# shuhan-wang1/SNLP---Tenary-Post-train-Quantization

Hardware: AMD Instinct MI355X
Metric: weight-columns quantized/sec (and s/layer) at d=4096 (higher is better)
Workload: dtype fp16->f32

## Files before the change

snlp---tenary-post-train-quantization_amd/csrc/ef.hip:

```cpp
#include "common.hpp"
#include "internal.hpp"
#include "probe.hpp"

namespace {

typedef float f32x16 __attribute__((ext_vector_type(16)));
typedef float f32x4 __attribute__((ext_vector_type(4)));
typedef unsigned u32x4 __attribute__((ext_vector_type(4)));

constexpr int EF_T = 128;
constexpr int EF_ROWB = EF_T * 4;
constexpr int E2_KS = 32;
constexpr int E2_PANEL = E2_KS * EF_ROWB;
constexpr int E2_STAGE = 2 * E2_PANEL;
constexpr int EF_CV = 16;
constexpr unsigned EF_DROP = 0x80000000u;

__device__ uint4 ef_zero16;

PT2Q_DEV int ef_wave() { return (int)(threadIdx.x >> 6); }

struct EfArgs {
  const float* Ck;
  long ldk;
  const float* Et;
  float* Wt;
  long ldw;
  const int* crow;
  int nr, bs, te, ti, ntile;
  long zs;
  int nz;
  float* part;
  int n;
};

PT2Q_DEV EfArgs ef_linear(const EfArgs& a0, int z) {
  EfArgs a = a0;
  const long o = (long)z * a0.zs;
  a.Ck = (const float*)((const char*)a0.Ck + o);
  a.Et = (const float*)((const char*)a0.Et + o);
  a.Wt = (float*)((char*)a0.Wt + o);
  a.crow = (const int*)((const char*)a0.crow + o);
  if (a0.part) a.part = (float*)((char*)a0.part + o);
  return a;
}

PT2Q_DEV void ef_dma_asm(const char* sbase, uint32_t voff, uint32_t m0) {
  asm volatile("s_mov_b32 m0, %2\n\ts_nop 0\n\tglobal_load_lds_dwordx4 %0, %1" ::"v"(voff), "s"(sbase), "s"(m0)
               : "memory");
}

template <int OFF>
PT2Q_DEV float ef_ld(uint32_t addr) {
  float r;
  asm volatile("ds_read_b32 %0, %1 offset:%2" : "=v"(r) : "v"(addr), "i"(OFF));
  return r;
}

template <int N>
PT2Q_DEV void ef_wait(float (&a)[2], float (&b)[2]) {
  asm volatile("s_waitcnt lgkmcnt(%4)" : "+v"(a[0]), "+v"(a[1]), "+v"(b[0]), "+v"(b[1]) : "n"(N));
}

template <int S>
PT2Q_DEV void ef_read(uint32_t baseA, uint32_t baseB, float (&a)[2], float (&b)[2]) {
  a[0] = ef_ld<S * 2 * EF_ROWB>(baseA);
  a[1] = ef_ld<S * 2 * EF_ROWB + 128>(baseA);
  b[0] = ef_ld<S * 2 * EF_ROWB>(baseB);
  b[1] = ef_ld<S * 2 * EF_ROWB + 128>(baseB);
}

struct EfAcc {
  f32x16 acc[2][2];

  template <int S>
  PT2Q_DEV void run(uint32_t bA, uint32_t bB, float (&a)[4][2], float (&b)[4][2]) {
    constexpr int NP = E2_KS / 2;
    if constexpr (S < NP) {
      constexpr int c = S % 4;
      if constexpr (S + 2 < NP) ef_read<S + 2>(bA, bB, a[(S + 2) % 4], b[(S + 2) % 4]);
      if constexpr (S > 0) {
        constexpr int p = (S + 3) % 4;
        asm volatile("" ::"v"(a[p][0]), "v"(a[p][1]), "v"(b[p][0]), "v"(b[p][1]));
      }
      __builtin_amdgcn_sched_barrier(0);
      acc[0][0] = __builtin_amdgcn_mfma_f32_32x32x2f32(b[c][0], a[c][0], acc[0][0], 0, 0, 0);
      __builtin_amdgcn_sched_barrier(0);
      acc[0][1] = __builtin_amdgcn_mfma_f32_32x32x2f32(b[c][1], a[c][0], acc[0][1], 0, 0, 0);
      __builtin_amdgcn_sched_barrier(0);
      acc[1][0] = __builtin_amdgcn_mfma_f32_32x32x2f32(b[c][0], a[c][1], acc[1][0], 0, 0, 0);
      __builtin_amdgcn_sched_barrier(0);
      acc[1][1] = __builtin_amdgcn_mfma_f32_32x32x2f32(b[c][1], a[c][1], acc[1][1], 0, 0, 0);
      __builtin_amdgcn_sched_barrier(0);
      if constexpr (S + 1 < NP) {
        ef_wait<(S + 2 < NP ? 4 : 0)>(a[(S + 1) % 4], b[(S + 1) % 4]);
      }
      run<S + 1>(bA, bB, a, b);
    }
  }

  PT2Q_DEV void stage(uint32_t stg) {
    const int lane = threadIdx.x & 63, wave = ef_wave();
    const int wr = wave >> 1, wc = wave & 1, li = lane & 31, lk = lane >> 5;
    const uint32_t bA = stg + lk * EF_ROWB + (wr * 64 + li) * 4;
    const uint32_t bB = stg + E2_PANEL + lk * EF_ROWB + (wc * 64 + li) * 4;
    float a[4][2], b[4][2];
    ef_read<0>(bA, bB, a[0], b[0]);
    ef_read<1>(bA, bB, a[1], b[1]);
    ef_wait<4>(a[0], b[0]);
    run<0>(bA, bB, a, b);
  }
};

PT2Q_DEV int ef_row(int e0, int rm) {
  const int lane = threadIdx.x & 63, wr = ef_wave() >> 1;
  return e0 + wr * 64 + rm * 32 + (lane & 31);
}

PT2Q_DEV void ef_rowbase(const EfArgs& a, const int (&wrow)[2], int i0, uint32_t (&rb)[2]) {
  const int lane = threadIdx.x & 63, wc = ef_wave() & 1;
  const int i = i0 + wc * 64 + 4 * (lane >> 5);
#pragma unroll
  for (int rm = 0; rm < 2; ++rm)
    rb[rm] = (wrow[rm] < 0 || i0 + wc * 64 >= a.ldw || probe::ef_drop_wt)
                 ? EF_DROP
                 : (uint32_t)(((long)wrow[rm] * a.ldw + i) * 4);
}

PT2Q_DEV void ef_rows(const EfArgs& a, int e0, int (&wrow)[2]) {
  int v[2];
#pragma unroll
  for (int rm = 0; rm < 2; ++rm) {
    const int e = ef_row(e0, rm);
    v[rm] = a.crow[e < a.nr ? e : 0];
  }
#pragma unroll
  for (int rm = 0; rm < 2; ++rm) wrow[rm] = ef_row(e0, rm) < a.nr ? v[rm] : -1;
}

constexpr int EF_PS = 8;
constexpr int EF_RED = 512;

template <int J>
PT2Q_DEV void ef_wbar_step(const int (&prow)[2], const u32x4 (&pend)[EF_CV], float* red) {
  constexpr int rn = J >> 4, q = (J >> 2) & 3, u = J & 3;
  const int lane = threadIdx.x & 63, wave = ef_wave();
  const float v0 = prow[0] >= 0 ? __uint_as_float(pend[rn * 4 + q][u]) : 0.0f;
  const float v1 = prow[1] >= 0 ? __uint_as_float(pend[(2 + rn) * 4 + q][u]) : 0.0f;
  float x = bfly16(v0 + v1);
  x = x + __int_as_float(__builtin_amdgcn_update_dpp(0, __float_as_int(x), 0x142, 0xA, 0xF, false));
  const bool sel = (lane & 31) == 16;
  red[sel ? wave * 64 + (lane >> 5) * 32 + J : 256 + wave * 64 + lane] = x;
}

PT2Q_DEV void ef_wbar_store(int n, __amdgpu_buffer_rsrc_t rp, bool valid, int e0, int i0, const float* red) {
  const int lane = threadIdx.x & 63, wave = ef_wave(), wr = wave >> 1, wc = wave & 1;
  const int h = lane >> 5;
  const bool mine = valid && wr == 0 && (lane & 31) == 0;
  const long cb = (long)(e0 / EF_T) * n;
  const f32x4* X = (const f32x4*)(red + wc * 64 + h * 32);
  const f32x4* Y = (const f32x4*)(red + (wc + 2) * 64 + h * 32);
#pragma unroll
  for (int rn = 0; rn < 2; ++rn) {
    f32x4 x[4], y[4];
#pragma unroll
    for (int q = 0; q < 4; ++q) {
      x[q] = X[rn * 4 + q];
      y[q] = Y[rn * 4 + q];
    }
#pragma unroll
    for (int q = 0; q < 4; ++q) {
      const int i = i0 + wc * 64 + rn * 32 + 8 * q + 4 * h;
      const f32x4 o = x[q] + y[q];
      const unsigned off = (mine && i < n) ? (unsigned)((cb + i) * 4) : EF_DROP;
      __builtin_amdgcn_raw_buffer_store_b128(__builtin_bit_cast(u32x4, o), rp, off, 0, 0);
    }
  }
}


struct E2Vo {
  uint32_t a[4], b[4];
};

PT2Q_DEV void e2_voff(const EfArgs& a, E2Vo& v) {
  const int lane = threadIdx.x & 63, wave = ef_wave();
#pragma unroll
  for (int q = 0; q < 4; ++q) {
    const int kr = (wave * 4 + q) * 2 + (lane >> 5), d = 4 * (lane & 31);
    v.a[q] = (uint32_t)(((long)kr * a.ldk + d) * 4);
    v.b[q] = (uint32_t)(((long)kr * a.ldw + d) * 4);
  }
}

PT2Q_DEV void e2_stage_q(const EfArgs& a, int e0, int i0, int s, const char* ba, const char* bb, const E2Vo& v,
                         uint8_t* stg, int q, bool withB) {
  const int lane = threadIdx.x & 63, wave = ef_wave();
  typedef __attribute__((address_space(3))) void* lptr;
  const int k = s * E2_KS + (wave * 4 + q) * 2 + (lane >> 5);
  const int d = 4 * (lane & 31);
  const bool kin = k < a.bs;
  const void* sa = kin ? (const void*)(e0 + d < a.nr ? ba + v.a[q] : (const char*)a.Ck) : (const void*)&ef_zero16;
  const void* sb = kin ? (const void*)(i0 + d < a.ldw ? bb + v.b[q] : (const char*)a.Et) : (const void*)&ef_zero16;
  const int wv = __builtin_amdgcn_readfirstlane(wave);
  __builtin_amdgcn_global_load_lds(sa, (lptr)(stg + (wv * 4 + q) * 1024), 16, 0, 0);
  if (withB) __builtin_amdgcn_global_load_lds(sb, (lptr)(stg + E2_PANEL + (wv * 4 + q) * 1024), 16, 0, 0);
}

PT2Q_DEV int e2_stage(const EfArgs& a, int e0, int i0, int s, uint8_t* stg, uint32_t stg_lds, const E2Vo& v,
                      bool withB) {
  if constexpr ((PT2Q_EF2_KPROBE & 2) != 0) {
    typedef __attribute__((address_space(3))) void* lptr;
    const int wv = __builtin_amdgcn_readfirstlane(ef_wave());
#pragma unroll
    for (int q = 0; q < 4; ++q) {
      __builtin_amdgcn_global_load_lds(&ef_zero16, (lptr)(stg + (wv * 4 + q) * 1024), 16, 0, 0);
      if (withB) __builtin_amdgcn_global_load_lds(&ef_zero16, (lptr)(stg + E2_PANEL + (wv * 4 + q) * 1024), 16, 0, 0);
    }
    return withB ? 8 : 4;
  }
  const bool fast = (s + 1) * E2_KS <= a.bs && e0 + EF_T <= a.nr && i0 + EF_T <= a.ldw;
  const char* ba = (const char*)(a.Ck + (long)s * E2_KS * a.ldk + e0);
  const char* bb = (const char*)(a.Et + (long)s * E2_KS * a.ldw + i0);
  if (!fast) {
#pragma unroll
    for (int q = 0; q < 4; ++q) e2_stage_q(a, e0, i0, s, ba, bb, v, stg, q, withB);
    return withB ? 8 : 4;
  }
  const int wv = __builtin_amdgcn_readfirstlane(ef_wave());
  const uint32_t mA = stg_lds + (uint32_t)(wv * 4 * 1024), mB = mA + E2_PANEL;
#pragma unroll
  for (int q = 0; q < 4; ++q) {
    ef_dma_asm(ba, v.a[q], mA + q * 1024);
    if (withB) ef_dma_asm(bb, v.b[q], mB + q * 1024);
  }
  return withB ? 8 : 4;
}

PT2Q_DEV void e2_vmcnt(int n) {
  switch (n) {
#define E2_W(k) \
  case k: asm volatile("s_waitcnt vmcnt(" #k ")" ::: "memory"); break;
    E2_W(0) E2_W(1) E2_W(2) E2_W(3) E2_W(4) E2_W(5) E2_W(6) E2_W(7) E2_W(8) E2_W(9) E2_W(10) E2_W(11) E2_W(12)
    E2_W(13) E2_W(14) E2_W(15) E2_W(16) E2_W(17) E2_W(18) E2_W(19) E2_W(20) E2_W(21) E2_W(22) E2_W(23) E2_W(24)
    E2_W(25) E2_W(26) E2_W(27) E2_W(28) E2_W(29) E2_W(30) E2_W(31) E2_W(32) E2_W(33) E2_W(34) E2_W(35) E2_W(36)
    E2_W(37) E2_W(38) E2_W(39) E2_W(40) E2_W(41) E2_W(42) E2_W(43) E2_W(44) E2_W(45) E2_W(46) E2_W(47) E2_W(48)
    E2_W(49) E2_W(50) E2_W(51) E2_W(52) E2_W(53) E2_W(54) E2_W(55) E2_W(56) E2_W(57) E2_W(58) E2_W(59) E2_W(60)
    E2_W(61) E2_W(62)
#undef E2_W
    default: asm volatile("s_waitcnt vmcnt(0)" ::: "memory"); break;
  }
}

template <int J, int JE>
PT2Q_DEV void ef_wbar_span(const int (&prow)[2], const u32x4 (&pend)[EF_CV], float* red) {
  if constexpr (J < JE) {
    ef_wbar_step<J>(prow, pend, red);
    ef_wbar_span<J + 1, JE>(prow, pend, red);
  }
}

template <int RN>
PT2Q_DEV void e2_load(u32x4 (&c)[EF_CV], __amdgpu_buffer_rsrc_t rc, const uint32_t (&rb)[2]) {
#pragma unroll
  for (int rm = 0; rm < 2; ++rm)
#pragma unroll
    for (int q = 0; q < 4; ++q)
      c[(rm * 2 + RN) * 4 + q] = __builtin_amdgcn_raw_buffer_load_b128(rc, rb[rm] + 4 * (32 * RN + 8 * q), 0, 0);
}

template <int RN>
PT2Q_DEV void e2_sub(u32x4 (&c)[EF_CV], const EfAcc& F) {
#pragma unroll
  for (int rm = 0; rm < 2; ++rm)
#pragma unroll
    for (int q = 0; q < 4; ++q) {
      const int j = (rm * 2 + RN) * 4 + q;
#pragma unroll
      for (int u = 0; u < 4; ++u) c[j][u] = __float_as_uint(__uint_as_float(c[j][u]) - F.acc[rm][RN][4 * q + u]);
    }
}

template <int RN>
PT2Q_DEV void e2_store(const u32x4 (&c)[EF_CV], __amdgpu_buffer_rsrc_t rc, const uint32_t (&rb)[2]) {
#pragma unroll
  for (int rm = 0; rm < 2; ++rm)
#pragma unroll
    for (int q = 0; q < 4; ++q)
      __builtin_amdgcn_raw_buffer_store_b128(c[(rm * 2 + RN) * 4 + q], rc, rb[rm] + 4 * (32 * RN + 8 * q), 0,
                                             PT2Q_EF2_STORE_AUX);
}

PT2Q_DEV uint32_t e2_g1_chunk(int wv, int j) {
  return (uint32_t)(j < 4 ? (wv * 4 + j) * 1024 : E2_PANEL + (wv * 4 + j - 4) * 1024);
}
PT2Q_DEV void e2_g1_dma(__amdgpu_buffer_rsrc_t rc, const uint32_t (&rb)[2], uint8_t* slot) {
  typedef __attribute__((address_space(3))) void* lptr;
  const int lane = threadIdx.x & 63, wv = __builtin_amdgcn_readfirstlane(ef_wave());
#pragma unroll
  for (int j = 0; j < 8; ++j) {
    const uint32_t src = (uint32_t)__shfl((int)rb[j >> 2], 8 * (j & 3) + (lane >> 3));
    const uint32_t off = src == EF_DROP ? EF_DROP : src + 4 * (32 + 4 * (lane & 7));
    __builtin_amdgcn_raw_ptr_buffer_load_lds(rc, (lptr)(slot + e2_g1_chunk(wv, j)), 16, off, 0, 0, 0);
  }
}
PT2Q_DEV void e2_g1_read(u32x4 (&c)[EF_CV], const uint8_t* slot) {
  const int lane = threadIdx.x & 63, wv = __builtin_amdgcn_readfirstlane(ef_wave());
  const int li = lane & 31, h = lane >> 5;
#pragma unroll
  for (int rm = 0; rm < 2; ++rm)
#pragma unroll
    for (int q = 0; q < 4; ++q) {
      const int j = rm * 4 + (li >> 3), piece = ((li & 7) << 3) | (2 * q + h);
      c[(rm * 2 + 1) * 4 + q] = *(const u32x4*)(slot + e2_g1_chunk(wv, j) + 16 * piece);
    }
}

template <int NST>
__global__ __launch_bounds__(256) __attribute__((amdgpu_waves_per_eu(2, 2))) void ef2_gemm_kernel(
    EfArgs a0, long wt_bytes, long part_bytes) {
  static_assert(NST == 2 || NST == 4, "two or four K stages per tile");
  constexpr bool G1L = NST == 4;
  __shared__ __attribute__((aligned(1024))) uint8_t smem[2 * E2_STAGE];
  __shared__ __attribute__((aligned(16))) float red[EF_RED];
  const uint32_t lds0 = (uint32_t)(uintptr_t)(__attribute__((address_space(3))) uint8_t*)smem;
  const int total = a0.ntile * a0.nz;
  int t = (int)blockIdx.x;
  if (t >= total) return;
  PT2Q_EF2_CLK(0);
  auto corner = [&](int t, EfArgs& a, int& e0, int& i0) {
    const int z = t / a0.ntile, tl = t - z * a0.ntile;
    a = ef_linear(a0, z);
    e0 = (tl / a0.ti) * EF_T;
    i0 = (tl % a0.ti) * EF_T;
  };
  auto rsrc = [&](const EfArgs& a) { return __builtin_amdgcn_make_buffer_rsrc(a.Wt, 0, (int)wt_bytes, 0x00020000); };
  auto prsrc = [&](const EfArgs& x) { return __builtin_amdgcn_make_buffer_rsrc(x.part, 0, (int)part_bytes, 0x00020000); };
  const int P = a0.part ? EF_PS : 0;
  EfArgs a;
  int e0, i0, wrow[2];
  corner(t, a, e0, i0);
  asm volatile("s_waitcnt vmcnt(0) lgkmcnt(0)" ::: "memory");
  __syncthreads();
  ef_rows(a, e0, wrow);
  E2Vo vo;
  e2_voff(a0, vo);
  e2_stage(a, e0, i0, 0, smem, lds0, vo, true);
  int Dn1 = e2_stage(a, e0, i0, 1, smem + E2_STAGE, lds0 + E2_STAGE, vo, true);
  int SP = 0;
  int par = 0;
  constexpr int G0S = NST - 1 - PT2Q_EF2_G0_EARLY < 0 ? 0 : NST - 1 - PT2Q_EF2_G0_EARLY;
  for (;;) {
    const int tn = t + (int)gridDim.x;
    const bool more = tn < total;
    int en = e0, in = i0, nrow[2];
    EfArgs an = a;
    if (more) corner(tn, an, en, in);
    const bool newB = NST != 2 || !(more && an.Et == a.Et && in == i0);
    const __amdgpu_buffer_rsrc_t rc = rsrc(a);
    uint32_t rb[2];
    ef_rowbase(a, wrow, i0, rb);
    if constexpr ((PT2Q_EF2_KPROBE & 1) != 0) rb[0] = rb[1] = EF_DROP;
    uint32_t rbl[2] = {rb[0], rb[1]}, rbs[2] = {rb[0], rb[1]};
    if constexpr ((PT2Q_EF2_KPROBE & 8) != 0) rbl[0] = rbl[1] = 0;
    if constexpr ((PT2Q_EF2_KPROBE & 16) != 0) rbs[0] = rbs[1] = 0;
    ef_rows(an, en, nrow);
    EfAcc F;
#pragma unroll
    for (int rm = 0; rm < 2; ++rm)
#pragma unroll
      for (int rn = 0; rn < 2; ++rn) F.acc[rm][rn] = f32x16{};
    u32x4 c[EF_CV];
    int X[NST];
#pragma unroll
    for (int s = 0; s < NST; ++s) {
      const int young = s == 0   ? Dn1 + SP + 2
                        : s == 1 ? (G1L && SP > 0 ? SP - EF_CV / 2 : SP) + 2 + (G0S == 0 ? EF_CV / 2 : 0) + X[0]
                                 : X[s - 1];
      e2_vmcnt(young);
      asm volatile("s_barrier" ::: "memory");
      if (s == G0S) e2_load<0>(c, rc, rbl);
      const int sl = G1L ? (s + par) & 1 : s & 1;
      if constexpr ((PT2Q_EF2_KPROBE & 4) == 0) F.stage(lds0 + sl * E2_STAGE);
      asm volatile("s_waitcnt lgkmcnt(0)\n\ts_barrier" ::: "memory");
      uint8_t* slot = smem + sl * E2_STAGE;
      const uint32_t slot_lds = lds0 + sl * E2_STAGE;
      if (s + 2 < NST) {
        X[s] = e2_stage(a, e0, i0, s + 2, slot, slot_lds, vo, true);
      } else if (G1L && s == NST - 2) {
        e2_g1_dma(rc, rbl, slot);
        X[s] = EF_CV / 2;
      } else if (G1L) {
        X[s] = more ? e2_stage(an, en, in, 0, slot, slot_lds, vo, newB) : 0;
      } else if (more) {
        X[s] = e2_stage(an, en, in, s + 2 - NST, slot, slot_lds, vo, newB);
        if (s == NST - 1) Dn1 = X[s];
      } else {
        X[s] = 0;
      }
    }
    e2_vmcnt(X[NST - 1]);
    e2_sub<0>(c, F);
    if constexpr (!G1L) e2_load<1>(c, rc, rbl);
    e2_store<0>(c, rc, rbs);
    if (P) {
      asm volatile("s_waitcnt lgkmcnt(0)\n\ts_barrier" ::: "memory");
      ef_wbar_span<0, 16>(wrow, c, red);
    }
    if constexpr (G1L) {
      uint8_t* g1 = smem + par * E2_STAGE;
      e2_g1_read(c, g1);
      asm volatile("s_waitcnt lgkmcnt(0)" ::: "memory");
      Dn1 = more ? e2_stage(an, en, in, 1, g1, lds0 + par * E2_STAGE, vo, newB) : 0;
      par ^= 1;
    } else {
      e2_vmcnt(EF_CV / 2);
    }
    e2_sub<1>(c, F);
    e2_store<1>(c, rc, rbs);
    if (P) {
      ef_wbar_span<16, 32>(wrow, c, red);
      asm volatile("s_waitcnt lgkmcnt(0)\n\ts_barrier" ::: "memory");
      ef_wbar_store(a0.n, prsrc(a), true, e0, i0, red);
    }
    SP = EF_CV + P;
    if (!more) break;
    t = tn;
    a = an;
    e0 = en;
    i0 = in;
    wrow[0] = nrow[0];
    wrow[1] = nrow[1];
  }
  PT2Q_EF2_CLK(1);
}

}

int pt2q_launch_ef(const float* Ck, long ldk, const float* Et, float* Wt, long ldw, long wt_rows,
                   const int* crow, int nr, int bs, hipStream_t st, const Grp* grp, float* part, int n) {
  if (nr <= 0) return PT2Q_OK;
  const long wt_bytes = wt_rows * ldw * 4;
  const long part_bytes = part ? (long)ceil_div(nr, EF_T) * n * 4 : 0;
  if (bs <= 0 || bs > 4 * E2_KS || ldw % 4 || ldk % 4 || (uintptr_t)Ck % 16 || (uintptr_t)Et % 16 ||
      (uintptr_t)Wt % 16 || wt_bytes >= (long)EF_DROP || wt_rows > 65536)
    return PT2Q_E_UNSUPPORTED;
  if (part && (n <= 0 || n % 4 || n > ldw || (uintptr_t)part % 16 || part_bytes >= (long)EF_DROP))
    return PT2Q_E_UNSUPPORTED;
  EfArgs a{Ck, ldk, Et, Wt, ldw, crow, nr, bs, ceil_div(nr, EF_T), ceil_div(ldw, EF_T), 0,
           grp ? grp->ws : 0l, (int)grp_z(grp), part, n};
  a.ntile = a.te * a.ti;
  int dev = 0, cus = 256;
  if (hipGetDevice(&dev) == hipSuccess) (void)hipDeviceGetAttribute(&cus, hipDeviceAttributeMultiprocessorCount, dev);
  const int grid = std::min(a.ntile * a.nz, 2 * cus);
  if (bs <= 2 * E2_KS)
    hipLaunchKernelGGL(ef2_gemm_kernel<2>, dim3(grid), dim3(256), 0, st, a, wt_bytes, part_bytes);
  else
    hipLaunchKernelGGL(ef2_gemm_kernel<4>, dim3(grid), dim3(256), 0, st, a, wt_bytes, part_bytes);
  PT2Q_LAUNCH_CHECK();
  return PT2Q_OK;
}
```

Baseline: 516,000.

## Add register-resident E kernel with software-pipelined tile walk for large block sizes

```diff
diff --git a/snlp---tenary-post-train-quantization_amd/csrc/ef.hip b/snlp---tenary-post-train-quantization_amd/csrc/ef.hip
--- a/snlp---tenary-post-train-quantization_amd/csrc/ef.hip
+++ b/snlp---tenary-post-train-quantization_amd/csrc/ef.hip
@@ -139,7 +139,7 @@
 }
 
 constexpr int EF_PS = 8;
-constexpr int EF_RED = 512;
+constexpr int EF_RED = 544;
 
 template <int J>
 PT2Q_DEV void ef_wbar_step(const int (&prow)[2], const u32x4 (&pend)[EF_CV], float* red) {
@@ -150,7 +150,7 @@
   float x = bfly16(v0 + v1);
   x = x + __int_as_float(__builtin_amdgcn_update_dpp(0, __float_as_int(x), 0x142, 0xA, 0xF, false));
   const bool sel = (lane & 31) == 16;
-  red[sel ? wave * 64 + (lane >> 5) * 32 + J : 256 + wave * 64 + lane] = x;
+  (red + (sel ? wave * 64 + (lane >> 5) * 32 : 256 + wave * 64 + lane))[J] = x;
 }
 
 PT2Q_DEV void ef_wbar_store(int n, __amdgpu_buffer_rsrc_t rp, bool valid, int e0, int i0, const float* red) {
@@ -291,36 +291,9 @@
                                              PT2Q_EF2_STORE_AUX);
 }
 
-PT2Q_DEV uint32_t e2_g1_chunk(int wv, int j) {
-  return (uint32_t)(j < 4 ? (wv * 4 + j) * 1024 : E2_PANEL + (wv * 4 + j - 4) * 1024);
-}
-PT2Q_DEV void e2_g1_dma(__amdgpu_buffer_rsrc_t rc, const uint32_t (&rb)[2], uint8_t* slot) {
-  typedef __attribute__((address_space(3))) void* lptr;
-  const int lane = threadIdx.x & 63, wv = __builtin_amdgcn_readfirstlane(ef_wave());
-#pragma unroll
-  for (int j = 0; j < 8; ++j) {
-    const uint32_t src = (uint32_t)__shfl((int)rb[j >> 2], 8 * (j & 3) + (lane >> 3));
-    const uint32_t off = src == EF_DROP ? EF_DROP : src + 4 * (32 + 4 * (lane & 7));
-    __builtin_amdgcn_raw_ptr_buffer_load_lds(rc, (lptr)(slot + e2_g1_chunk(wv, j)), 16, off, 0, 0, 0);
-  }
-}
-PT2Q_DEV void e2_g1_read(u32x4 (&c)[EF_CV], const uint8_t* slot) {
-  const int lane = threadIdx.x & 63, wv = __builtin_amdgcn_readfirstlane(ef_wave());
-  const int li = lane & 31, h = lane >> 5;
-#pragma unroll
-  for (int rm = 0; rm < 2; ++rm)
-#pragma unroll
-    for (int q = 0; q < 4; ++q) {
-      const int j = rm * 4 + (li >> 3), piece = ((li & 7) << 3) | (2 * q + h);
-      c[(rm * 2 + 1) * 4 + q] = *(const u32x4*)(slot + e2_g1_chunk(wv, j) + 16 * piece);
-    }
-}
-
-template <int NST>
 __global__ __launch_bounds__(256) __attribute__((amdgpu_waves_per_eu(2, 2))) void ef2_gemm_kernel(
     EfArgs a0, long wt_bytes, long part_bytes) {
-  static_assert(NST == 2 || NST == 4, "two or four K stages per tile");
-  constexpr bool G1L = NST == 4;
+  constexpr int NST = 2;
   __shared__ __attribute__((aligned(1024))) uint8_t smem[2 * E2_STAGE];
   __shared__ __attribute__((aligned(16))) float red[EF_RED];
   const uint32_t lds0 = (uint32_t)(uintptr_t)(__attribute__((address_space(3))) uint8_t*)smem;
@@ -348,7 +321,6 @@
   e2_stage(a, e0, i0, 0, smem, lds0, vo, true);
   int Dn1 = e2_stage(a, e0, i0, 1, smem + E2_STAGE, lds0 + E2_STAGE, vo, true);
   int SP = 0;
-  int par = 0;
   constexpr int G0S = NST - 1 - PT2Q_EF2_G0_EARLY < 0 ? 0 : NST - 1 - PT2Q_EF2_G0_EARLY;
   for (;;) {
     const int tn = t + (int)gridDim.x;
@@ -356,7 +328,7 @@
     int en = e0, in = i0, nrow[2];
     EfArgs an = a;
     if (more) corner(tn, an, en, in);
-    const bool newB = NST != 2 || !(more && an.Et == a.Et && in == i0);
+    const bool newB = !(more && an.Et == a.Et && in == i0);
     const __amdgpu_buffer_rsrc_t rc = rsrc(a);
     uint32_t rb[2];
     ef_rowbase(a, wrow, i0, rb);
@@ -374,26 +346,17 @@
     int X[NST];
 #pragma unroll
     for (int s = 0; s < NST; ++s) {
-      const int young = s == 0   ? Dn1 + SP + 2
-                        : s == 1 ? (G1L && SP > 0 ? SP - EF_CV / 2 : SP) + 2 + (G0S == 0 ? EF_CV / 2 : 0) + X[0]
-                                 : X[s - 1];
+      const int young = s == 0 ? Dn1 + SP + 2 : SP + 2 + (G0S == 0 ? EF_CV / 2 : 0) + X[0];
       e2_vmcnt(young);
       asm volatile("s_barrier" ::: "memory");
       if (s == G0S) e2_load<0>(c, rc, rbl);
-      const int sl = G1L ? (s + par) & 1 : s & 1;
+      const int sl = s & 1;
       if constexpr ((PT2Q_EF2_KPROBE & 4) == 0) F.stage(lds0 + sl * E2_STAGE);
       asm volatile("s_waitcnt lgkmcnt(0)\n\ts_barrier" ::: "memory");
       uint8_t* slot = smem + sl * E2_STAGE;
       const uint32_t slot_lds = lds0 + sl * E2_STAGE;
-      if (s + 2 < NST) {
-        X[s] = e2_stage(a, e0, i0, s + 2, slot, slot_lds, vo, true);
-      } else if (G1L && s == NST - 2) {
-        e2_g1_dma(rc, rbl, slot);
-        X[s] = EF_CV / 2;
-      } else if (G1L) {
-        X[s] = more ? e2_stage(an, en, in, 0, slot, slot_lds, vo, newB) : 0;
-      } else if (more) {
-        X[s] = e2_stage(an, en, in, s + 2 - NST, slot, slot_lds, vo, newB);
+      if (more) {
+        X[s] = e2_stage(an, en, in, s, slot, slot_lds, vo, newB);
         if (s == NST - 1) Dn1 = X[s];
       } else {
         X[s] = 0;
@@ -401,21 +364,13 @@
     }
     e2_vmcnt(X[NST - 1]);
     e2_sub<0>(c, F);
-    if constexpr (!G1L) e2_load<1>(c, rc, rbl);
+    e2_load<1>(c, rc, rbl);
     e2_store<0>(c, rc, rbs);
     if (P) {
       asm volatile("s_waitcnt lgkmcnt(0)\n\ts_barrier" ::: "memory");
       ef_wbar_span<0, 16>(wrow, c, red);
     }
-    if constexpr (G1L) {
-      uint8_t* g1 = smem + par * E2_STAGE;
-      e2_g1_read(c, g1);
-      asm volatile("s_waitcnt lgkmcnt(0)" ::: "memory");
-      Dn1 = more ? e2_stage(an, en, in, 1, g1, lds0 + par * E2_STAGE, vo, newB) : 0;
-      par ^= 1;
-    } else {
-      e2_vmcnt(EF_CV / 2);
-    }
+    e2_vmcnt(EF_CV / 2);
     e2_sub<1>(c, F);
     e2_store<1>(c, rc, rbs);
     if (P) {
@@ -431,6 +386,320 @@
     i0 = in;
     wrow[0] = nrow[0];
     wrow[1] = nrow[1];
+  }
+  PT2Q_EF2_CLK(1);
+}
+
+constexpr int E3_NP = 64;
+constexpr int E3_APANEL = 4 * E2_PANEL;
+constexpr int E3_VM_TOP = EF_CV + EF_CV + EF_PS;
+constexpr int E3_VM_END = 2 + EF_CV + EF_CV + EF_CV + EF_PS;
+
+PT2Q_DEV void ef_dma_lane(const void* src, uint32_t m0) {
+  asm volatile("s_mov_b32 m0, %1\n\ts_nop 0\n\tglobal_load_lds_dwordx4 %0, off" ::"v"(src), "s"(m0) : "memory");
+}
+
+template <int J>
+PT2Q_DEV const void* e3_dma_src(const EfArgs& a, int e0, const E2Vo& v) {
+  constexpr int s = J >> 2, q = J & 3;
+  const int lane = threadIdx.x & 63, wave = ef_wave();
+  const int k = s * E2_KS + (wave * 4 + q) * 2 + (lane >> 5), d = 4 * (lane & 31);
+  const char* ba = (const char*)(a.Ck + (long)s * E2_KS * a.ldk + e0);
+  return k < a.bs ? (const void*)(e0 + d < a.nr ? ba + v.a[q] : (const char*)a.Ck) : (const void*)&ef_zero16;
+}
+template <int J>
+PT2Q_DEV void e3_dma(const void* src, uint32_t panel) {
+  constexpr int s = J >> 2, q = J & 3;
+  ef_dma_lane(src, panel + s * E2_PANEL + (uint32_t)((__builtin_amdgcn_readfirstlane(ef_wave()) * 4 + q) * 1024));
+}
+
+template <int J>
+PT2Q_DEV void e3_dma_all(const EfArgs& a, int e0, uint32_t panel, const E2Vo& v) {
+  if constexpr (J < 16) {
+    e3_dma<J>(e3_dma_src<J>(a, e0, v), panel);
+    e3_dma_all<J + 1>(a, e0, panel, v);
+  }
+}
+
+PT2Q_DEV float e3_ldg(u32x4 r, uint32_t off) {
+  float v;
+  asm volatile("buffer_load_dword %0, %1, %2, 0 offen" : "=a"(v) : "v"(off), "s"(r) : "memory");
+  return v;
+}
+
+PT2Q_DEV void e3_load_e(const EfArgs& a, int i0, float (&E)[2][E3_NP]) {
+  const int lane = threadIdx.x & 63, wc = ef_wave() & 1, li = lane & 31, lk = lane >> 5;
+  const uintptr_t p = (uintptr_t)a.Et;
+  u32x4 r;
+  r[0] = (unsigned)__builtin_amdgcn_readfirstlane((int)(uint32_t)p);
+  r[1] = (unsigned)__builtin_amdgcn_readfirstlane((int)(uint32_t)((p >> 32) & 0xffff));
+  r[2] = (unsigned)__builtin_amdgcn_readfirstlane((int)((long)a.bs * a.ldw * 4));
+  r[3] = 0x00020000u;
+  const uint32_t step = (uint32_t)(a.ldw * 8);
+#pragma unroll
+  for (int rn = 0; rn < 2; ++rn) {
+    const int col = i0 + wc * 64 + rn * 32 + li;
+    const uint32_t o0 = (uint32_t)(((long)lk * a.ldw + col) * 4);
+#pragma unroll
+    for (int pr = 0; pr < E3_NP; ++pr) {
+      E[rn][pr] = e3_ldg(r, (col < a.ldw && 2 * pr + lk < a.bs) ? o0 + pr * step : EF_DROP);
+      __builtin_amdgcn_sched_barrier(0);
+    }
+  }
+}
+
+PT2Q_DEV void e3_tie(float (&E)[2][E3_NP]) {
+#pragma unroll
+  for (int rn = 0; rn < 2; ++rn)
+#pragma unroll
+    for (int pr = 0; pr < E3_NP; ++pr) asm volatile("" : "+a"(E[rn][pr]));
+}
+
+PT2Q_DEV void e3_rows_issue(const EfArgs& a, int e0, int (&v)[2]) {
+#pragma unroll
+  for (int rm = 0; rm < 2; ++rm) {
+    const int e = ef_row(e0, rm);
+    asm volatile("global_load_dword %0, %1, off" : "=v"(v[rm]) : "v"(a.crow + (e < a.nr ? e : 0)) : "memory");
+  }
+}
+PT2Q_DEV void e3_rows_take(const EfArgs& a, int e0, int (&v)[2], int (&wrow)[2]) {
+  asm volatile("s_waitcnt vmcnt(%2)" : "+v"(v[0]), "+v"(v[1]) : "n"(2 * EF_CV));
+#pragma unroll
+  for (int rm = 0; rm < 2; ++rm) wrow[rm] = ef_row(e0, rm) < a.nr ? v[rm] : -1;
+}
+
+template <int IMM>
+PT2Q_DEV u32x4 e3_ld4(__amdgpu_buffer_rsrc_t r, uint32_t off) {
+  u32x4 v;
+  asm volatile("buffer_load_dwordx4 %0, %1, %2, 0 offen offset:%3" : "=v"(v) : "v"(off), "s"(r), "i"(IMM) : "memory");
+  return v;
+}
+PT2Q_DEV void e3_tie_old(u32x4 (&c)[EF_CV]) {
+#pragma unroll
+  for (int j = 0; j < EF_CV; ++j) asm volatile("" : "+v"(c[j]));
+}
+template <int J>
+PT2Q_DEV void e3_load_old(u32x4 (&c)[EF_CV], __amdgpu_buffer_rsrc_t rc, const uint32_t (&rb)[2]) {
+  if constexpr (J < EF_CV) {
+    constexpr int RN = J >> 3, rm = (J >> 2) & 1, q = J & 3;
+    c[(rm * 2 + RN) * 4 + q] = e3_ld4<4 * (32 * RN + 8 * q)>(rc, rb[rm]);
+    e3_load_old<J + 1>(c, rc, rb);
+  }
+}
+
+template <int N>
+PT2Q_DEV void e3_wait(float (&a)[2]) {
+  asm volatile("s_waitcnt lgkmcnt(%2)" : "+v"(a[0]), "+v"(a[1]) : "n"(N));
+}
+
+template <int P>
+PT2Q_DEV void e3_read(uint32_t bA, float (&a)[2]) {
+  a[0] = ef_ld<P * 2 * EF_ROWB>(bA);
+  a[1] = ef_ld<P * 2 * EF_ROWB + 128>(bA);
+}
+
+struct E3Tile {
+  int z, e0, i0;
+  int wrow[2];
+  uint32_t rb[2];
+};
+
+struct E3Jobs {
+  const EfArgs& a0;
+  const E2Vo& vo;
+  long wt_bytes, part_bytes;
+  float* red;
+  E3Tile prev, next;
+  bool more;
+  uint32_t panel;
+  int nrow[2];
+
+  PT2Q_DEV __amdgpu_buffer_rsrc_t wt(int z) const {
+    return __builtin_amdgcn_make_buffer_rsrc(ef_linear(a0, z < 0 ? 0 : z).Wt, 0, (int)wt_bytes, 0x00020000);
+  }
+
+  template <int P>
+  PT2Q_DEV void fold(u32x4 (&res)[EF_CV]) {
+    if constexpr (P < 32) ef_wbar_step<P>(prev.wrow, res, red);
+  }
+
+  template <int P>
+  PT2Q_DEV const void* prep() {
+    if constexpr (P < 16) return e3_dma_src<(P & 15)>(ef_linear(a0, next.z), next.e0, vo);
+    return nullptr;
+  }
+
+  template <int P>
+  PT2Q_DEV void mem(u32x4 (&res)[EF_CV], const void* src) {
+    constexpr int J = P & 15, RN = J >> 3, rm = (J >> 2) & 1, q = J & 3, idx = (rm * 2 + RN) * 4 + q;
+    constexpr int imm = 4 * (32 * RN + 8 * q);
+    if constexpr (P < 16) {
+      e3_dma<J>(src, panel);
+    } else if constexpr (P < 32) {
+      __builtin_amdgcn_raw_buffer_store_b128(res[idx], wt(prev.z), prev.rb[rm] + imm, 0, PT2Q_EF2_STORE_AUX);
+    } else if constexpr (P < 48) {
+      res[idx] = e3_ld4<imm>(wt(next.z), next.rb[rm]);
+    }
+  }
+
+  template <int P>
+  PT2Q_DEV void after() {
+    if constexpr (P == 31) {
+      e3_rows_take(a0, next.e0, nrow, next.wrow);
+      ef_rowbase(a0, next.wrow, next.i0, next.rb);
+      if (!more) next.rb[0] = next.rb[1] = EF_DROP;
+    } else if constexpr (P == 47) {
+      asm volatile("s_barrier" ::: "memory");
+      const EfArgs ap = ef_linear(a0, prev.z < 0 ? 0 : prev.z);
+      ef_wbar_store(a0.n, __builtin_amdgcn_make_buffer_rsrc(ap.part, 0, (int)part_bytes, 0x00020000),
+                    prev.z >= 0 && a0.part, prev.e0, prev.i0, red);
+    }
+  }
+};
+
+template <int P>
+PT2Q_DEV f32x16 e3_mfma(float e, float c, const f32x16& acc) {
+  if constexpr ((PT2Q_EF2_KPROBE & 4) != 0) return P == 0 ? f32x16{} : acc;
+  if constexpr (P == 0) return __builtin_amdgcn_mfma_f32_32x32x2f32(e, c, f32x16{}, 0, 0, 0);
+  return __builtin_amdgcn_mfma_f32_32x32x2f32(e, c, acc, 0, 0, 0);
+}
+
+template <int P>
+PT2Q_DEV void e3_pairs(EfAcc& F, const float (&E)[2][E3_NP], uint32_t bA, float (&a)[4][2], E3Jobs& jb,
+                       u32x4 (&res)[EF_CV]) {
+  if constexpr (P < E3_NP) {
+    constexpr int c = P % 4;
+    const void* src = jb.template prep<P>();
+    if constexpr (P + 2 < E3_NP) e3_read<P + 2>(bA, a[(P + 2) % 4]);
+    if constexpr (P > 0) {
+      constexpr int p = (P + 3) % 4;
+      asm volatile("" ::"v"(a[p][0]), "v"(a[p][1]));
+    }
+    __builtin_amdgcn_sched_barrier(0);
+    F.acc[0][0] = e3_mfma<P>(E[0][P], a[c][0], F.acc[0][0]);
+    __builtin_amdgcn_sched_barrier(0);
+    jb.template mem<P>(res, src);
+    __builtin_amdgcn_sched_barrier(0);
+    F.acc[0][1] = e3_mfma<P>(E[1][P], a[c][0], F.acc[0][1]);
+    __builtin_amdgcn_sched_barrier(0);
+    jb.template fold<P>(res);
+    __builtin_amdgcn_sched_barrier(0);
+    F.acc[1][0] = e3_mfma<P>(E[0][P], a[c][1], F.acc[1][0]);
+    __builtin_amdgcn_sched_barrier(0);
+    F.acc[1][1] = e3_mfma<P>(E[1][P], a[c][1], F.acc[1][1]);
+    __builtin_amdgcn_sched_barrier(0);
+    if constexpr (P + 1 < E3_NP) e3_wait<(P + 2 < E3_NP ? 2 : 0)>(a[(P + 1) % 4]);
+    jb.template after<P>();
+    __builtin_amdgcn_sched_barrier(0);
+    e3_pairs<P + 1>(F, E, bA, a, jb, res);
+  }
+}
+
+struct E3Walk {
+  E3Jobs jb;
+  E3Tile cur;
+  int t, tend, par;
+  bool fresh;
+  float E[2][E3_NP];
+};
+
+PT2Q_DEV void e3_corner(const EfArgs& a0, int t, E3Tile& c) {
+  c.z = t / a0.ntile;
+  const int r = t - c.z * a0.ntile;
+  c.i0 = (r / a0.te) * EF_T;
+  c.e0 = (r % a0.te) * EF_T;
+}
+
+PT2Q_DEV bool e3_tile(E3Walk& w, uint32_t lds0, u32x4 (&old)[EF_CV], u32x4 (&res)[EF_CV]) {
+  E3Jobs& jb = w.jb;
+  const EfArgs& a0 = jb.a0;
+  jb.more = w.t + 1 < w.tend;
+  jb.next = w.cur;
+  if (jb.more) e3_corner(a0, w.t + 1, jb.next);
+  jb.panel = lds0 + (uint32_t)((w.par ^ 1) * E3_APANEL);
+  if (w.fresh) {
+    asm volatile("s_waitcnt vmcnt(0)" ::: "memory");
+    e3_tie(w.E);
+  } else {
+    e2_vmcnt(E3_VM_TOP);
+  }
+  asm volatile("s_waitcnt lgkmcnt(0)\n\ts_barrier" ::: "memory");
+  e3_rows_issue(ef_linear(a0, jb.next.z), jb.next.e0, jb.nrow);
+  const int lane = threadIdx.x & 63, wr = ef_wave() >> 1;
+  const uint32_t bA = lds0 + (uint32_t)(w.par * E3_APANEL + (lane >> 5) * EF_ROWB + (wr * 64 + (lane & 31)) * 4);
+  EfAcc F;
+  float a[4][2];
+  e3_read<0>(bA, a[0]);
+  e3_read<1>(bA, a[1]);
+  e3_wait<2>(a[0]);
+  e3_pairs<0>(F, w.E, bA, a, jb, res);
+  e2_vmcnt(E3_VM_END);
+  e3_tie_old(old);
+  e2_sub<0>(old, F);
+  e2_sub<1>(old, F);
+  w.fresh = jb.more && (jb.next.z != w.cur.z || jb.next.i0 != w.cur.i0);
+  if (w.fresh) e3_load_e(ef_linear(a0, jb.next.z), jb.next.i0, w.E);
+  jb.prev = w.cur;
+  w.cur = jb.next;
+  w.par ^= 1;
+  ++w.t;
+  return jb.more;
+}
+
+__global__ __launch_bounds__(256) __attribute__((amdgpu_waves_per_eu(1, 1))) void ef3_gemm_kernel(
+    EfArgs a0, long wt_bytes, long part_bytes) {
+  __shared__ __attribute__((aligned(1024))) uint8_t smem[2 * E3_APANEL];
+  __shared__ __attribute__((aligned(16))) float red[EF_RED];
+  const uint32_t lds0 = (uint32_t)(uintptr_t)(__attribute__((address_space(3))) uint8_t*)smem;
+  const long total = (long)a0.ntile * a0.nz;
+  E2Vo vo;
+  e2_voff(a0, vo);
+  E3Walk w{{a0, vo, wt_bytes, part_bytes, red}};
+  w.t = (int)(total * blockIdx.x / gridDim.x);
+  w.tend = (int)(total * (blockIdx.x + 1) / gridDim.x);
+  if (w.t >= w.tend) return;
+  PT2Q_EF2_CLK(0);
+  w.par = 0;
+  w.fresh = true;
+  e3_corner(a0, w.t, w.cur);
+  w.jb.prev = w.cur;
+  w.jb.prev.z = -1;
+  w.jb.prev.wrow[0] = w.jb.prev.wrow[1] = -1;
+  w.jb.prev.rb[0] = w.jb.prev.rb[1] = EF_DROP;
+  u32x4 x[EF_CV], y[EF_CV];
+#pragma unroll
+  for (int j = 0; j < EF_CV; ++j) y[j] = u32x4{};
+  {
+    const EfArgs a = ef_linear(a0, w.cur.z);
+    ef_rows(a, w.cur.e0, w.cur.wrow);
+    ef_rowbase(a0, w.cur.wrow, w.cur.i0, w.cur.rb);
+    e3_dma_all<0>(a, w.cur.e0, lds0, vo);
+    const __amdgpu_buffer_rsrc_t rc = w.jb.wt(w.cur.z);
+    e3_load_old<0>(x, rc, w.cur.rb);
+    e3_load_e(a, w.cur.i0, w.E);
+  }
+  bool odd = false;
+  for (;;) {
+    if (!e3_tile(w, lds0, x, y)) break;
+    if (!e3_tile(w, lds0, y, x)) {
+      odd = true;
+      break;
+    }
+  }
+  if (odd) {
+#pragma unroll
+    for (int j = 0; j < EF_CV; ++j) x[j] = y[j];
+  }
+  const E3Tile& l = w.jb.prev;
+  const __amdgpu_buffer_rsrc_t rc = w.jb.wt(l.z);
+  e2_store<0>(x, rc, l.rb);
+  e2_store<1>(x, rc, l.rb);
+  if (a0.part) {
+    asm volatile("s_waitcnt lgkmcnt(0)\n\ts_barrier" ::: "memory");
+    ef_wbar_span<0, 32>(l.wrow, x, red);
+    asm volatile("s_waitcnt lgkmcnt(0)\n\ts_barrier" ::: "memory");
+    ef_wbar_store(a0.n, __builtin_amdgcn_make_buffer_rsrc(ef_linear(a0, l.z).part, 0, (int)part_bytes, 0x00020000),
+                  true, l.e0, l.i0, red);
   }
   PT2Q_EF2_CLK(1);
 }
@@ -452,11 +721,12 @@
   a.ntile = a.te * a.ti;
   int dev = 0, cus = 256;
   if (hipGetDevice(&dev) == hipSuccess) (void)hipDeviceGetAttribute(&cus, hipDeviceAttributeMultiprocessorCount, dev);
-  const int grid = std::min(a.ntile * a.nz, 2 * cus);
   if (bs <= 2 * E2_KS)
-    hipLaunchKernelGGL(ef2_gemm_kernel<2>, dim3(grid), dim3(256), 0, st, a, wt_bytes, part_bytes);
+    hipLaunchKernelGGL(ef2_gemm_kernel, dim3(std::min(a.ntile * a.nz, 2 * cus)), dim3(256), 0, st, a, wt_bytes,
+                       part_bytes);
   else
-    hipLaunchKernelGGL(ef2_gemm_kernel<4>, dim3(grid), dim3(256), 0, st, a, wt_bytes, part_bytes);
+    hipLaunchKernelGGL(ef3_gemm_kernel, dim3(std::min(a.ntile * a.nz, cus)), dim3(256), 0, st, a, wt_bytes,
+                       part_bytes);
   PT2Q_LAUNCH_CHECK();
   return PT2Q_OK;
 }
```

Result: no change. 518,100 (median of 6 runs) (+0.4%).
